# Yotsuei/ClearConverse

Hardware: AMD Instinct MI355X
Metric: xRT (audio-sec/wall-sec) end-to-end, 30 s 16 kHz clips (higher is better)
Workload: dtype bf16

## Files before the change

### clearconverse_amd/_lib.py

```python
from __future__ import annotations

import ctypes as C
import os
from pathlib import Path
from typing import Optional

_PKG = Path(__file__).resolve().parent
LIB_PATH = _PKG / "libccx.so"


class CcxError(RuntimeError):
    pass


class WhisperDims(C.Structure):
    _fields_ = [(n, C.c_int) for n in (
        "n_mels", "n_audio_ctx", "n_audio_state", "n_audio_head", "n_audio_layer",
        "n_vocab", "n_text_ctx", "n_text_state", "n_text_head", "n_text_layer")]


class SepformerDims(C.Structure):
    _fields_ = [(n, C.c_int) for n in (
        "n_filters", "kernel", "stride", "d_model", "n_head", "d_ffn", "n_layers", "n_blocks", "segment", "n_spk")]

# ... 41 lines not shown


class DecSeqState(C.Structure):
    _fields_ = [(n, C.c_int) for n in ("pos", "prompt_len", "n_gen", "done", "last_tok", "pen_tok", "last_ts_tok", "n_tokens")] + [
        ("sum_logprob", C.c_float), ("no_speech_prob", C.c_float)]


class DecSelectDesc(C.Structure):
    _fields_ = [
        ("logits", C.c_void_p), ("ld", C.c_int64), ("n_vocab", C.c_int), ("B", C.c_int),
        ("rules", C.POINTER(DecodeRules)), ("state", C.POINTER(DecSeqState)),
        ("prompt", C.POINTER(C.c_int)), ("max_prompt", C.c_int), ("sample_len", C.c_int),
        ("gen", C.POINTER(C.c_int)), ("cur_tok", C.POINTER(C.c_int)), ("pos", C.POINTER(C.c_int)), ("n_done", C.POINTER(C.c_int)),
        ("tok_emb", C.c_void_p), ("pos_emb", C.c_void_p), ("x", C.c_void_p), ("D", C.c_int),
        ("sample", C.c_int), ("temperature", C.c_float), ("seed", C.c_uint64), ("row0", C.c_int),
        ("logits_elems", C.c_int64), ("tok_emb_elems", C.c_int64), ("pos_emb_elems", C.c_int64), ("x_elems", C.c_int64),
        ("stream_ids", C.POINTER(C.c_int))]


class DecBeamDesc(C.Structure):
    _fields_ = [
        ("logits", C.c_void_p), ("ld", C.c_int64), ("n_vocab", C.c_int),
        ("G", C.c_int), ("beam_size", C.c_int), ("max_candidates", C.c_int),
        ("rules", C.POINTER(DecodeRules)), ("state", C.POINTER(DecSeqState)), ("sample_len", C.c_int),
        ("hist", C.POINTER(C.c_int)), ("cur_tok", C.POINTER(C.c_int)), ("pos", C.POINTER(C.c_int)), ("n_done", C.POINTER(C.c_int)),
        ("tok_emb", C.c_void_p), ("pos_emb", C.c_void_p), ("x", C.c_void_p), ("D", C.c_int),
        ("ind", C.POINTER(C.c_uint16)), ("ind_ld", C.c_int),
        ("fin_tok", C.POINTER(C.c_int)), ("fin_score", C.POINTER(C.c_float)), ("fin_n", C.POINTER(C.c_int)),
        ("fin_count", C.POINTER(C.c_int)),
        ("cand_id", C.POINTER(C.c_int)), ("cand_lp", C.POINTER(C.c_float)), ("tok_out", C.POINTER(C.c_int)),
        ("parent_out", C.POINTER(C.c_int)),
        ("logits_elems", C.c_int64), ("tok_emb_elems", C.c_int64), ("pos_emb_elems", C.c_int64), ("x_elems", C.c_int64)]


class BeamTrace(C.Structure):
    _fields_ = [("n_steps", C.c_int), ("cand_id", C.POINTER(C.c_int32)), ("cand_lp", C.POINTER(C.c_float)),
                ("tok", C.POINTER(C.c_int32)), ("parent", C.POINTER(C.c_int32)), ("score", C.POINTER(C.c_float))]


class DecTokenProbsDesc(C.Structure):
    _fields_ = [
        ("logits", C.c_void_p), ("logits_elems", C.c_int64), ("ld", C.c_int64), ("n_vocab", C.c_int), ("rows", C.c_int),
        ("lo", C.c_int), ("hi", C.c_int), ("pick", C.c_int),
        ("argmax", C.POINTER(C.c_int)), ("pick_prob", C.POINTER(C.c_float)),
        ("probs", C.c_void_p), ("probs_elems", C.c_int64)]


class DecPickProbsDesc(C.Structure):
    _fields_ = [
        ("logits", C.c_void_p), ("logits_elems", C.c_int64), ("ld", C.c_int64), ("rows", C.c_int), ("hi", C.c_int),
        ("picks", C.c_void_p), ("picks_elems", C.c_int64), ("pick_stride", C.c_int64),
        ("out", C.c_void_p), ("out_elems", C.c_int64), ("out_stride", C.c_int64)]


class SepDesc(C.Structure):
    _fields_ = (
        [(n, C.c_void_p) for n in ("h", "xin", "y", "qkv", "att", "feats", "fc")]
        + [(n, C.c_int64) for n in ("h_elems", "xin_elems", "y_elems", "qkv_elems", "att_elems", "feats_elems", "fc_elems")]
        + [("rows", C.c_int), ("seq_start", C.POINTER(C.c_int)), ("seq_len", C.POINTER(C.c_int)), ("n_seq", C.c_int),
           ("n_tok", C.c_int), ("d_ffn", C.c_int)]
        + [(n, C.c_void_p) for n in ("ln_g", "ln_b", "gln_g", "gln_b", "wqkv", "bqkv", "wo", "bo", "w1", "b1", "w2", "b2", "wdec")]
        + [(n, C.c_int64) for n in ("ln_elems", "gln_elems", "wqkv_elems", "bqkv_elems", "wo_elems", "bo_elems", "w1_elems",
                                    "b1_elems", "w2_elems", "b2_elems", "wdec_elems")]
        + [("utt_tok0", C.POINTER(C.c_int)), ("utt_L", C.POINTER(C.c_int)), ("utt_T", C.POINTER(C.c_int)), ("n_utt", C.c_int),
           ("segment", C.c_int), ("out", C.c_void_p), ("out_stride", C.c_int64), ("out_elems", C.c_int64)])


SEP_ATTN_BLOCK, SEP_ATTENTION, SEP_FFN, SEP_FINAL_NORM, SEP_DECODER = range(5)


class AlignDesc(C.Structure):
    _fields_ = [
        ("q", C.c_void_p), ("k", C.c_void_p), ("q_elems", C.c_int64), ("k_elems", C.c_int64),
        ("n_seq", C.c_int), ("H", C.c_int), ("Spad", C.c_int),
        ("heads", C.POINTER(C.c_int)), ("n_heads", C.c_int), ("head0", C.c_int), ("t", C.c_int),
        ("Hsel", C.c_int), ("T", C.c_int), ("Mmax", C.c_int),
        ("n_keys", C.POINTER(C.c_int)), ("n_rows", C.POINTER(C.c_int)), ("r0", C.c_int),
        ("P", C.c_void_p), ("A", C.c_void_p), ("P_elems", C.c_int64), ("A_elems", C.c_int64),
        ("text_idx", C.c_void_p), ("time_idx", C.c_void_p), ("path_len", C.c_void_p), ("jump_frame", C.c_void_p),
        ("text_idx_elems", C.c_int64), ("time_idx_elems", C.c_int64), ("path_len_elems", C.c_int64), ("jump_frame_elems", C.c_int64)]


ALIGN_SCORES, ALIGN_MATRIX, ALIGN_DTW = range(3)


_vp, _i, _i64, _f = C.c_void_p, C.c_int, C.c_int64, C.c_float
_ip = C.POINTER(C.c_int)
_i32p = C.POINTER(C.c_int32)
_i64p = C.POINTER(C.c_int64)
_fp = C.POINTER(C.c_float)

PROTOTYPES = {
    "ccx_version": (C.c_char_p, []),
    "ccx_ctx_create": (_i, [_i, C.POINTER(_vp)]),
    "ccx_ctx_destroy": (None, [_vp]),
    "ccx_last_error": (C.c_char_p, [_vp]),
    "ccx_prof_enable": (_i, [_vp, _i]),
    "ccx_prof_count": (_i, [_vp]),
    "ccx_prof_get": (_i, [_vp, _i, C.c_char_p, _i, C.POINTER(C.c_double), C.POINTER(C.c_double), _fp]),
    "ccx_gemm_bf16": (_i, [_vp, _i, _vp, _i64, _vp, _i64, _vp, _vp, _i64, _vp, _i64, _i, _i, _i, _vp]),
    "ccx_gemm_bf16_desc": (_i, [_vp, _i, C.POINTER(GemmDesc), _vp]),
    "ccx_layernorm": (_i, [_vp, _vp, _vp, _vp, _vp, _vp, _i, _i, _f, _vp]),
    "ccx_gather_rows": (_i, [_vp, _vp, _vp, _i, _i, _vp, _i64, _vp]),
    "ccx_peak_normalize": (_i, [_vp, _vp, _vp, _i64, _vp, _i, _f, _vp]),
    "ccx_row_variance": (_i, [_vp, _vp, _i64, _vp, _i, _vp, _vp]),
    "ccx_cross_attention_xa": (_i, [_vp, _vp, _vp, _vp, _vp, _vp, _vp, _i, _i, _i, _i, _i, _vp, _vp]),
    "ccx_cosine_rows": (_i, [_vp, _vp, _vp, _i, _i, _i, _vp, _vp]),
    "ccx_speaker_profiles": (_i, [_vp, _vp, _vp, _vp, _i, _i, _i, _i, _vp, _vp]),
    "ccx_resample_sinc": (_i, [_vp, _vp, _i64, _vp, _i, _i, _i, _i, _vp, _vp, _i64, _vp, _i, _vp]),
    "ccx_enc_attention": (_i, [_vp, _vp, _vp, _vp, _vp, _i, _i, _i, _i, _vp]),
    "ccx_whisper_create": (_i, [_vp, C.POINTER(WhisperDims), _i, C.POINTER(_vp)]),
    "ccx_whisper_destroy": (None, [_vp]),
    "ccx_whisper_set_tensor": (_i, [_vp, C.c_char_p, _vp, _i, _i, _i64p]),
    "ccx_whisper_set_max_audio": (_i, [_vp, C.c_double]),
    "ccx_whisper_share_encoder_scratch": (_i, [_vp, _vp]),
    "ccx_whisper_finalize": (_i, [_vp]),
    "ccx_whisper_set_rules": (_i, [_vp, C.POINTER(DecodeRules)]),
    "ccx_whisper_logmel": (_i, [_vp, _vp, _i64, _ip, _ip, _i, _vp, _vp]),
    "ccx_whisper_set_mel": (_i, [_vp, _vp, _i, _vp]),
    "ccx_whisper_encode": (_i, [_vp, _i, _vp, _vp]),
    "ccx_whisper_decoder_logits": (_i, [_vp, _i32p, _i, _i, _vp, _vp]),
    "ccx_whisper_decode_greedy": (_i, [_vp, _i32p, _i32p, _i, _i, _i, _i32p, _i32p, _fp, _fp, _vp]),
    "ccx_dec_attention_desc": (_i, [_vp, _i, C.POINTER(DecAttnDesc), _vp]),
    "ccx_dec_select_step": (_i, [_vp, C.POINTER(DecSelectDesc), _vp]),
    "ccx_dec_beam_step": (_i, [_vp, C.POINTER(DecBeamDesc), _vp]),
    "ccx_whisper_decode_beam": (_i, [_vp, _i32p, _i32p, _i, _i, _i32p, _i, _i, _i, _i, _i32p, _i32p, _fp, _i32p, _fp,
                                     C.POINTER(BeamTrace), _vp]),
    "ccx_dec_token_probs": (_i, [_vp, C.POINTER(DecTokenProbsDesc), _vp]),
    "ccx_dec_pick_probs": (_i, [_vp, C.POINTER(DecPickProbsDesc), _vp]),
    "ccx_align_op": (_i, [_vp, _i, C.POINTER(AlignDesc), _vp]),
    "ccx_whisper_align": (_i, [_vp, _i32p, _i32p, _i, _i, _i32p, _i32p, _i, _i, _vp, _vp, _i32p, _vp]),
    "ccx_whisper_align_probs": (_i, [_vp, _i32p, _i32p, _i, _i, _i32p, _i32p, _i, _i, _vp, _vp, _i32p, _i, _fp, _vp]),
    "ccx_whisper_last_cross_path": (_i, [_vp]),
    "ccx_whisper_set_sot_tail": (_i, [_vp, _i]),
    "ccx_whisper_detect_language": (_i, [_vp, _i, _i, _i, _i32p, _fp, _vp]),
    "ccx_whisper_prepare_lanes": (_i, [_vp, _vp]),
    "ccx_whisper_trace_lanes": (_i, [_vp, C.c_char_p, _i]),
    "ccx_whisper_decode": (_i, [_vp, _i32p, _i32p, _i, _i, _i, _f, C.c_uint64, _i32p, _i32p, _fp, _fp, _vp]),
    "ccx_whisper_decode_rows": (_i, [_vp, _i32p, _i32p, _i, _i, _i32p, _i, _i32p, _i, _f, C.c_uint64, _i32p, _i32p, _fp, _fp, _vp]),
    "ccx_sepformer_create": (_i, [_vp, C.POINTER(SepformerDims), _i, _i, C.POINTER(_vp)]),
    "ccx_sepformer_destroy": (None, [_vp]),
    "ccx_sepformer_set_tensor": (_i, [_vp, C.c_char_p, _vp, _i64]),
    "ccx_sepformer_finalize": (_i, [_vp]),
    "ccx_sepformer_separate": (_i, [_vp, _vp, _i64, _ip, _i, _vp, _vp]),
    "ccx_sep_op": (_i, [_vp, _i, C.POINTER(SepDesc), _vp]),
    "ccx_speaker_create": (_i, [_vp, _i, _i, _i, _i, _i64, C.POINTER(_vp)]),
    "ccx_speaker_destroy": (None, [_vp]),
    "ccx_speaker_set_tensor": (_i, [_vp, C.c_char_p, _vp, _i64]),
    "ccx_speaker_finalize": (_i, [_vp]),
    "ccx_speaker_embed": (_i, [_vp, _vp, _i64p, _ip, _i, _vp, _i64p, _ip, _vp, _vp]),
    "ccx_speaker_segment": (_i, [_vp, _vp, _i64p, _ip, _i, _vp, _i64, _ip, _vp]),
    "ccx_resnet_create": (_i, [_vp, _i, _i64, _i, C.POINTER(_vp)]),
    "ccx_resnet_destroy": (None, [_vp]),
    "ccx_resnet_set_tensor": (_i, [_vp, C.c_char_p, _vp, _i64]),
    "ccx_resnet_finalize": (_i, [_vp]),
    "ccx_resnet_embed": (_i, [_vp, _vp, _i64, _i, _i, _vp, _i, _ip, _i, _vp, _vp]),
    "ccx_specgate_create": (_i, [_vp, _i64, _i, _i, C.POINTER(_vp)]),
    "ccx_specgate_destroy": (None, [_vp]),
    "ccx_specgate_reduce": (_i, [_vp, _vp, _i64, _ip, _i, _f, _vp, _vp]),
    "ccx_specgate_reduce_long": (_i, [_vp, _vp, _i64, _f, _vp, _vp]),
    "ccx_specgate_set_clip_noise": (_i, [_vp, _i]),
}

_lib: Optional[C.CDLL] = None


def load() -> C.CDLL:
    global _lib
    if _lib is not None:
        return _lib
    if not LIB_PATH.exists():
        raise CcxError(f"{LIB_PATH} is missing: run `python -m clearconverse_amd.build` "
                       "(there is no CPU fallback for the HIP path)")
    import torch
    try:
        lib = C.CDLL(str(LIB_PATH))
    except OSError as e:
        raise CcxError(f"cannot load {LIB_PATH}: {e}") from e
    for name, (res, args) in PROTOTYPES.items():
        try:
            fn = getattr(lib, name)
        except AttributeError as e:
            raise CcxError(f"libccx.so does not export {name}") from e
        fn.restype = res
        fn.argtypes = args
    _lib = lib
    return lib


class Context:

    def __init__(self, device: int = 0):
        self.lib = load()
        h = _vp()
        rc = self.lib.ccx_ctx_create(device, C.byref(h))
        if rc != 0:
            raise CcxError(f"ccx_ctx_create({device}) failed: {self.lib.ccx_last_error(None).decode()}")
        self.handle = h
        self.device = device

    def check(self, rc: int, what: str = ""):
        if rc != 0:
            raise CcxError(f"{what or 'ccx call'} failed ({rc}): {self.lib.ccx_last_error(self.handle).decode()}")

    prof_on = False

    def prof_enable(self, on: bool = True):
        self.check(self.lib.ccx_prof_enable(self.handle, 1 if on else 0), "ccx_prof_enable")
        self.prof_on = bool(on)

    def prof_records(self):
        out = []
        buf = C.create_string_buffer(64)
        fl, by, ms = C.c_double(), C.c_double(), C.c_float()
        for i in range(self.lib.ccx_prof_count(self.handle)):
            self.check(self.lib.ccx_prof_get(self.handle, i, buf, 64, C.byref(fl), C.byref(by), C.byref(ms)), "ccx_prof_get")
            out.append((buf.value.decode(), fl.value, by.value, ms.value))
        return out

    def close(self):
        if getattr(self, "handle", None):
            self.lib.ccx_ctx_destroy(self.handle)
            self.handle = None

    def __del__(self):
        try:
            self.close()
        except Exception:
            pass


def current_stream_ptr() -> int:
    import torch
    return int(torch.cuda.current_stream().cuda_stream)


def ptr(t) -> int:
    if t is None:
        return 0
# ... 4 lines not shown
```

### clearconverse_amd/csrc/resnet.hip

```cpp
#include <string>
#include <vector>
#include <math.h>
#include "../../include/ccx.h"
#include "ccx_common.h"
#include "gemm_bf16.h"
#include "model_store.h"

namespace {

constexpr int FB_LEN = 400, FB_SHIFT = 160, FB_NFFT = 512, FB_MELS = 80, FB_MELW = 64;
constexpr int RN_C0 = 32, RN_EMB = 256, RN_STAGES = 4;
constexpr int RN_BLOCKS[RN_STAGES] = {3, 4, 6, 3};

__global__ __launch_bounds__(256) void fbank_kernel(const float* __restrict__ wav, long stride, int T, const float* __restrict__ window,
                                                    const float2* __restrict__ twiddle, const float* __restrict__ melw,
                                                    const int* __restrict__ mel_start, const int* __restrict__ mel_len,
                                                    float* __restrict__ feats_t) {
  __shared__ float2 buf[4][FB_NFFT];
  __shared__ float2 tw[FB_NFFT / 2];
  const int lane = threadIdx.x & 63, wave = threadIdx.x >> 6;
  for (int i = threadIdx.x; i < FB_NFFT / 2; i += 256) tw[i] = twiddle[i];
  const int chunk = blockIdx.y;
  const int t = blockIdx.x * 4 + wave;
  const bool live = t < T;
// ... 133 lines not shown
      const int row = idx / ((TW + 2) * 4), rem = idx - row * (TW + 2) * 4;
      const int px = rem >> 2, q = rem & 3;
      stg[it] = make_uint4(0, 0, 0, 0);
      if (idx < NCH && x0 + px < Wp) stg[it] = *(const uint4*)(src + ((long)row * Wp + x0 + px) * 32 + q * 8);
    }
    if (HAS_RESID) {
#pragma unroll
      for (int pt = 0; pt < 4; pt++) {
        const int x = x0 + pt * 16 + l15;
        rres[pt] = make_uint4(0, 0, 0, 0);
        if (x < W) rres[pt] = *(const uint4*)(resid + (orow + x) * 32 + 8 * hq);
      }
    }
  };
  auto put = [&]() {
#pragma unroll
    for (int it = 0; it < NIT; it++) {
      const int idx = tid + 256 * it;
      const int row = idx / ((TW + 2) * 4), rem = idx - row * (TW + 2) * 4;
      const int px = rem >> 2, q = rem & 3;
      if (idx < NCH) *(uint4*)(tile + (row * (TW + 2) + px) * PITCH + q * 16) = stg[it];
    }
  };
  fetch(0);
  bf16x8 wf[9][2];
#pragma unroll
  for (int t = 0; t < 9; t++)
#pragma unroll
    for (int j = 0; j < 2; j++) {
      const int co = 8 * (l15 >> 2) + 4 * j + (l15 & 3);
      wf[t][j] = *(const bf16x8*)(wpk + (long)co * 384 + (t / 3) * 128 + (t % 3) * 32 + hq * 8);
    }
  float bv[8];
#pragma unroll
  for (int i = 0; i < 8; i++) bv[i] = bias[8 * hq + i];
  const int n_tiles = (W + TW - 1) / TW;
  for (int k = 0; k < n_tiles; k++) {
    const int x0 = k * TW;
    put();
    uint4 rcur[4];
    if (HAS_RESID) {
#pragma unroll
      for (int pt = 0; pt < 4; pt++) rcur[pt] = rres[pt];
    }
    __syncthreads();
    if (k + 1 < n_tiles) fetch(x0 + TW);
    f32x4 acc[4][2];
#pragma unroll
    for (int pt = 0; pt < 4; pt++)
#pragma unroll
      for (int j = 0; j < 2; j++) acc[pt][j] = (f32x4){0.f, 0.f, 0.f, 0.f};
#pragma unroll
    for (int t = 0; t < 9; t++) {
      const int kh = t / 3, kw = t % 3;
#pragma unroll
      for (int pt = 0; pt < 4; pt++) {
        const bf16x8 bfrag = *(const bf16x8*)(tile + ((wave + kh) * (TW + 2) + pt * 16 + l15 + kw) * PITCH + hq * 16);
#pragma unroll
        for (int j = 0; j < 2; j++) acc[pt][j] = __builtin_amdgcn_mfma_f32_16x16x32_bf16(wf[t][j], bfrag, acc[pt][j], 0, 0, 0);
      }
    }
#pragma unroll
    for (int pt = 0; pt < 4; pt++) {
      const int x = x0 + pt * 16 + l15;
      if (x >= W) continue;
      float v[8];
#pragma unroll
      for (int j = 0; j < 2; j++)
#pragma unroll
        for (int r = 0; r < 4; r++) v[4 * j + r] = acc[pt][j][r] + bv[4 * j + r];
      const long off = (orow + x) * 32 + 8 * hq;
      if (HAS_RESID) {
        const uint32_t rw[4] = {rcur[pt].x, rcur[pt].y, rcur[pt].z, rcur[pt].w};
#pragma unroll
        for (int i = 0; i < 4; i++) {
          v[2 * i] += __uint_as_float(rw[i] << 16);
          v[2 * i + 1] += __uint_as_float(rw[i] & 0xffff0000u);
        }
      }
      uint4 o;
      o.x = pack_bf16x2(fmaxf(v[0], 0.f), fmaxf(v[1], 0.f)); o.y = pack_bf16x2(fmaxf(v[2], 0.f), fmaxf(v[3], 0.f));
      o.z = pack_bf16x2(fmaxf(v[4], 0.f), fmaxf(v[5], 0.f)); o.w = pack_bf16x2(fmaxf(v[6], 0.f), fmaxf(v[7], 0.f));
      *(uint4*)(out + off) = o;
    }
    __syncthreads();
  }
}

__global__ __launch_bounds__(256) void tstp_kernel(const bf16_t* __restrict__ act, int W4, const int* __restrict__ mask_chunk,
                                                   const float* __restrict__ weights, int n_w, float* __restrict__ pooled) {
  const int h = blockIdx.x, j = blockIdx.y, c = threadIdx.x;
  const int chunk = mask_chunk ? mask_chunk[j] : j;
  const long Wp = W4 + 2;
  const bf16_t* base = act + (((long)chunk * 12 + h + 1) * Wp + 1) * 256 + c;
  const float* wj = weights ? weights + (long)j * n_w : nullptr;
  float v1 = 0.f, v2 = 0.f, sx = 0.f;
  const float scale = (float)n_w / (float)W4;
  for (int t = 0; t < W4; t++) {
    const float w = wj ? wj[min((int)floorf(t * scale), n_w - 1)] : 1.f;
    v1 += w; v2 += w * w;
    sx = fmaf(w, bf16_to_f32(base[(long)t * 256]), sx);
  }
  v1 += 1e-8f;
  const float mean = sx / v1;
  float sq = 0.f;
  for (int t = 0; t < W4; t++) {
    const float w = wj ? wj[min((int)floorf(t * scale), n_w - 1)] : 1.f;
    const float d = bf16_to_f32(base[(long)t * 256]) - mean;
    sq = fmaf(w, d * d, sq);
  }
  const float var = sq / (v1 - v2 / v1 + 1e-8f);
  float* o = pooled + (long)j * 5120;
  o[c * 10 + h] = mean;
  o[2560 + c * 10 + h] = sqrtf(var);
}

__global__ __launch_bounds__(256) void embed_linear_kernel(const float* __restrict__ pooled, const float* __restrict__ W,
                                                           const float* __restrict__ bias, float* __restrict__ out) {
  const int lane = threadIdx.x & 63, o = blockIdx.x * 4 + (threadIdx.x >> 6), j = blockIdx.y;
  const float4* p = (const float4*)(pooled + (long)j * 5120);
  const float4* w = (const float4*)(W + (long)o * 5120);
  float s = 0.f;
  for (int i = lane; i < 5120 / 4; i += 64) {
    const float4 a = p[i], b = w[i];
    s += a.x * b.x + a.y * b.y + a.z * b.z + a.w * b.w;
  }
  s = wave_reduce_sum(s);
  if (lane == 0) out[(long)j * RN_EMB + o] = s + bias[o];
}

struct Conv {
  bf16_t* W = nullptr;
  float* b = nullptr;
  int cin = 0, cout = 0, k = 3, stride = 1, Kpad = 0;
};
struct Block {
  Conv c1, c2, sc;
  bool has_sc = false;
};

}

struct ccx_resnet {
  ccx_ctx* ctx = nullptr;
  int max_chunks = 0, max_masks = 0, max_frames = 0;
  long max_samples = 0;
  bool finalized = false;
  ccx_dev_store store{"resnet"};
  float *window = nullptr, *melw = nullptr;
  float2* twiddle = nullptr;
  int *mel_start = nullptr, *mel_len = nullptr;
  float *c1w = nullptr, *c1b = nullptr, *segW = nullptr, *segb = nullptr;
  std::vector<Block> blocks;
  float *feats_t = nullptr, *fmean = nullptr, *pooled = nullptr;
  bf16_t* act[RN_STAGES][3] = {};
  size_t act_elems[RN_STAGES] = {};
  int* mask_chunk_dev = nullptr;
  std::vector<int> mask_host[4];
  int mask_slot = 0;
  int last_T = -1;
  int halo_chunks = 0;
};

namespace {

int bn_fold(ccx_resnet* r, const std::string& name, int c, std::vector<float>& scale, std::vector<float>& shift) {
  CCX_NEED(r->store, g, name + ".weight", c); CCX_NEED(r->store, be, name + ".bias", c);
  CCX_NEED(r->store, rm, name + ".running_mean", c); CCX_NEED(r->store, rv, name + ".running_var", c);
  scale.resize(c); shift.resize(c);
  for (int i = 0; i < c; i++) {
    scale[i] = g->data[i] / sqrtf(rv->data[i] + 1e-5f);
    shift[i] = be->data[i] - rm->data[i] * scale[i];
  }
  return CCX_OK;
}

int load_conv(ccx_resnet* r, const std::string& wname, const std::string& bnname, int cin, int cout, int k, int stride, Conv& cv) {
  CCX_NEED(r->store, w, wname, (int64_t)cout * cin * k * k);
  std::vector<float> sc, sh;
  CCX_TRY(bn_fold(r, bnname, cout, sc, sh));
  cv.cin = cin; cv.cout = cout; cv.k = k; cv.stride = stride;
  cv.Kpad = ccx_align(k * cin, 64);
  std::vector<bf16_t> packed((size_t)cout * k * cv.Kpad, 0);
  for (int o = 0; o < cout; o++)
    for (int c = 0; c < cin; c++)
      for (int kh = 0; kh < k; kh++)
        for (int kw = 0; kw < k; kw++)
          packed[((size_t)o * k + kh) * cv.Kpad + kw * cin + c] = ccx_host_f32_to_bf16(w->data[(((size_t)o * cin + c) * k + kh) * k + kw] * sc[o]);
  CCX_TRY(r->store.upload(&cv.W, packed));
  CCX_TRY(r->store.upload(&cv.b, sh));
  return CCX_OK;
}

__global__ __launch_bounds__(256) void halo_zero_kernel(bf16_t* b0, bf16_t* b1, bf16_t* b2, int c0, int H, long Wp, int C) {
  bf16_t* buf = blockIdx.z == 0 ? b0 : (blockIdx.z == 1 ? b1 : b2);
  const int y = blockIdx.x;
  bf16_t* row = buf + (((long)(c0 + blockIdx.y) * (H + 2) + y) * Wp) * C;
  const uint4 z = make_uint4(0, 0, 0, 0);
  if (y == 0 || y == H + 1) {
    const long n = Wp * C / 8;
    for (long i = threadIdx.x; i < n; i += 256) ((uint4*)row)[i] = z;
  } else {
    const int n = C / 8;
    for (int i = threadIdx.x; i < 2 * n; i += 256) {
      bf16_t* cell = i < n ? row : row + (Wp - 1) * C;
      ((uint4*)cell)[i < n ? i : i - n] = z;
    }
  }
}

struct StageDims { int H, W, C; long Wp; };
void stage_dims(int T, StageDims (&d)[RN_STAGES]) {
  int H = FB_MELS, W = T, C = RN_C0;
  for (int s = 0; s < RN_STAGES; s++) {
    d[s] = {H, W, C, (long)W + 2};
    H /= 2; W = (W - 1) / 2 + 1; C *= 2;
  }
}

int run_conv(ccx_resnet* r, const Conv& cv, int epi, const bf16_t* in, const StageDims& di, bf16_t* out, const StageDims& dn,
             const bf16_t* resid, int n_chunks, hipStream_t st) {
  if (cv.cin == 32 && cv.cout == 32 && cv.k == 3 && cv.stride == 1 && di.H % 4 == 0 && (epi == EPI_BF16_RELU || epi == EPI_BF16_ADD_RELU)) {
    const dim3 grid(1, di.H / 4, n_chunks);
    {
      ccx_prof_scope ps(r->ctx, st, "conv3x3_c32_kernel", 2.0 * 9 * 32 * 32 * (double)n_chunks * di.H * di.W,
                        (double)n_chunks * di.H * di.W * 64.0 * (resid ? 3 : 2));
      if (resid) hipLaunchKernelGGL(conv3x3_c32_kernel<true>, grid, dim3(256), 0, st, in, cv.W, cv.b, resid, out, di.H, di.W);
      else hipLaunchKernelGGL(conv3x3_c32_kernel<false>, grid, dim3(256), 0, st, in, cv.W, cv.b, resid, out, di.H, di.W);
    }
    CCX_CHECK_LAUNCH(r->ctx);
    return CCX_OK;
  }
  GemmParams p;
  memset(&p, 0, sizeof(p));
  const int s = cv.stride;
  const int RI = (di.H + 2) / s;
  p.A = in + (cv.k == 1 ? (di.Wp + 1) * di.C : 0);
  p.lda = (long)s * di.C;
  p.K = cv.Kpad; p.ntaps = cv.k; p.a_tap_stride = di.Wp * di.C;
  p.W = cv.W; p.ldw = (long)cv.k * cv.Kpad;
  p.M = (int)((long)n_chunks * RI * di.Wp); p.N = cv.cout;
  p.bias = cv.b; p.out = out; p.ldo = cv.cout;
  p.rpb_in = (int)di.Wp; p.rpb_valid = dn.W; p.rpb_out = (int)dn.Wp; p.roff = (int)dn.Wp + 1;
  p.img_rows_in = RI; p.img_rows_valid = dn.H; p.img_rows_out = dn.H + 2;
  p.resid_bf16 = resid; p.ldrb = cv.cout;
  return ccx_launch_gemm(r->ctx, epi, p, st);
}

}

extern "C" {

int ccx_resnet_create(ccx_ctx* ctx, int max_chunks, int64_t max_samples, int max_masks, ccx_resnet** out) {
  if (!ctx || !out) return CCX_ERR_ARG;
  CCX_REQUIRE(ctx, max_chunks >= 1 && max_masks >= 1 && max_samples >= FB_LEN + 7 * FB_SHIFT, "resnet_create: bad capacities");
  const int max_frames = 1 + (int)((max_samples - FB_LEN) / FB_SHIFT);
  CCX_REQUIRE(ctx, (long)max_chunks * 82 * (max_frames + 2) < (1L << 31), "resnet_create: max_chunks x frames too large for one launch");
  ccx_resnet* r = new ccx_resnet();
  r->ctx = ctx; r->store.ctx = ctx; r->max_chunks = max_chunks; r->max_masks = max_masks; r->max_samples = max_samples;
  r->max_frames = max_frames;
  *out = r;
  return CCX_OK;
}

void ccx_resnet_destroy(ccx_resnet* r) {
  if (!r) return;
  r->store.free_all();
  delete r;
}

int ccx_resnet_set_tensor(ccx_resnet* r, const char* name, const float* data, int64_t numel) {
  if (!r) return CCX_ERR_ARG;
  CCX_REQUIRE(r->ctx, !r->finalized && name && data && numel > 0, "resnet: set_tensor bad arguments");
  return r->store.stage(name, data, numel);
}

int ccx_resnet_finalize(ccx_resnet* r) {
  if (!r) return CCX_ERR_ARG;
  ccx_ctx* ctx = r->ctx;
  CCX_REQUIRE(ctx, !r->finalized, "resnet: finalize called twice");
  {
    std::vector<float> win(FB_LEN);
    for (int i = 0; i < FB_LEN; i++) win[i] = (float)(0.54 - 0.46 * cos(2.0 * M_PI * i / (FB_LEN - 1)));
    std::vector<float2> tw(FB_NFFT / 2);
    for (int i = 0; i < FB_NFFT / 2; i++) tw[i] = make_float2((float)cos(-2.0 * M_PI * i / FB_NFFT), (float)sin(-2.0 * M_PI * i / FB_NFFT));
    auto mel = [](double f) { return 1127.0 * log(1.0 + f / 700.0); };
    const double mlo = mel(20.0), mhi = mel(8000.0), delta = (mhi - mlo) / (FB_MELS + 1);
    std::vector<float> mw((size_t)FB_MELS * FB_MELW, 0.f);
    std::vector<int> ms(FB_MELS, 0), ml(FB_MELS, 0);
    for (int m = 0; m < FB_MELS; m++) {
      const double left = mlo + m * delta, center = left + delta, right = center + delta;
      int first = -1, last = -1;
      std::vector<float> wts(FB_NFFT / 2, 0.f);
      for (int k = 0; k < FB_NFFT / 2; k++) {
        const double mk = mel(16000.0 / FB_NFFT * k);
        const double up = (mk - left) / (center - left), down = (right - mk) / (right - center);
        const double wv = fmax(0.0, fmin(up, down));
        wts[k] = (float)wv;
        if (wv > 0.0) { if (first < 0) first = k; last = k; }
      }
      if (first < 0) { first = 0; last = -1; }
      CCX_REQUIRE(ctx, last - first + 1 <= FB_MELW, "resnet: mel filter %d spans %d bins", m, last - first + 1);
      ms[m] = first; ml[m] = last - first + 1;
      for (int k = first; k <= last; k++) mw[(size_t)m * FB_MELW + (k - first)] = wts[k];
    }
    CCX_TRY(r->store.upload(&r->window, win)); CCX_TRY(r->store.upload(&r->twiddle, tw)); CCX_TRY(r->store.upload(&r->melw, mw));
    CCX_TRY(r->store.upload(&r->mel_start, ms)); CCX_TRY(r->store.upload(&r->mel_len, ml));
  }
  {
    CCX_NEED(r->store, w, "resnet.conv1.weight", RN_C0 * 9);
    std::vector<float> sc, sh;
    CCX_TRY(bn_fold(r, "resnet.bn1", RN_C0, sc, sh));
    std::vector<float> wf(RN_C0 * 9);
    for (int c = 0; c < RN_C0; c++)
      for (int k = 0; k < 9; k++) wf[c * 9 + k] = w->data[c * 9 + k] * sc[c];
    CCX_TRY(r->store.upload(&r->c1w, wf)); CCX_TRY(r->store.upload(&r->c1b, sh));
  }
  int cin = RN_C0;
  for (int s = 0; s < RN_STAGES; s++) {
    const int cout = RN_C0 << s;
    for (int b = 0; b < RN_BLOCKS[s]; b++) {
      const std::string p = "resnet.layer" + std::to_string(s + 1) + "." + std::to_string(b) + ".";
      const int stride = (s > 0 && b == 0) ? 2 : 1;
      Block blk;
      CCX_TRY(load_conv(r, p + "conv1.weight", p + "bn1", cin, cout, 3, stride, blk.c1));
      CCX_TRY(load_conv(r, p + "conv2.weight", p + "bn2", cout, cout, 3, 1, blk.c2));
      blk.has_sc = stride != 1 || cin != cout;
      if (blk.has_sc) CCX_TRY(load_conv(r, p + "shortcut.0.weight", p + "shortcut.1", cin, cout, 1, stride, blk.sc));
      r->blocks.push_back(blk);
      cin = cout;
    }
  }
  {
    CCX_NEED(r->store, w, "resnet.seg_1.weight", (int64_t)RN_EMB * 5120); CCX_NEED(r->store, b, "resnet.seg_1.bias", RN_EMB);
    CCX_TRY(r->store.upload(&r->segW, w->data)); CCX_TRY(r->store.upload(&r->segb, b->data));
  }
  r->store.staged.clear();
  const int T = r->max_frames;
  CCX_TRY(r->store.alloc(&r->feats_t, (size_t)r->max_chunks * FB_MELS * T, true));
  CCX_TRY(r->store.alloc(&r->fmean, (size_t)r->max_chunks * FB_MELS, true));
  CCX_TRY(r->store.alloc(&r->pooled, (size_t)r->max_masks * 5120, true));
  CCX_TRY(r->store.alloc(&r->mask_chunk_dev, (size_t)r->max_masks, true));
  StageDims d[RN_STAGES];
  stage_dims(T, d);
  for (int s = 0; s < RN_STAGES; s++) {
    r->act_elems[s] = (size_t)r->max_chunks * (d[s].H + 2) * d[s].Wp * d[s].C + 4 * d[s].Wp * d[s].C + 1024;
    for (int k = 0; k < 3; k++) CCX_TRY(r->store.alloc(&r->act[s][k], r->act_elems[s], true));
  }
  r->finalized = true;
  return CCX_OK;
}

int ccx_resnet_embed(ccx_resnet* r, const float* wav_dev, int64_t stride, int n_samples, int n_chunks, const float* weights_dev,
                     int n_w, const int* mask_chunk, int n_masks, float* out_dev, void* stream_) {
  if (!r) return CCX_ERR_ARG;
  ccx_ctx* ctx = r->ctx;
  hipStream_t st = (hipStream_t)stream_;
  CCX_REQUIRE(ctx, r->finalized, "resnet: not finalized");
  CCX_REQUIRE(ctx, wav_dev && out_dev && n_chunks >= 1 && n_chunks <= r->max_chunks, "resnet_embed: bad chunk count %d (max %d)", n_chunks, r->max_chunks);
  CCX_REQUIRE(ctx, n_samples <= stride && n_samples <= r->max_samples, "resnet_embed: n_samples %d exceeds stride or capacity", n_samples);
  const int T = n_samples >= FB_LEN ? 1 + (n_samples - FB_LEN) / FB_SHIFT : 0;
  StageDims d[RN_STAGES];
  stage_dims(T > 0 ? T : 1, d);
  CCX_REQUIRE(ctx, T >= 1 && d[3].W >= 2, "resnet_embed: %d samples are too short (at least two pooled frames are needed)", n_samples);
  if (weights_dev) {
    CCX_REQUIRE(ctx, mask_chunk && n_masks >= 1 && n_masks <= r->max_masks && n_w >= 1, "resnet_embed: bad mask arguments");
    for (int j = 0; j < n_masks; j++)
      CCX_REQUIRE(ctx, mask_chunk[j] >= 0 && mask_chunk[j] < n_chunks, "resnet_embed: mask_chunk[%d]=%d out of range", j, mask_chunk[j]);
    std::vector<int>& keep = r->mask_host[r->mask_slot++ & 3];
    keep.assign(mask_chunk, mask_chunk + n_masks);
    CCX_HIP(ctx, hipMemcpyAsync(r->mask_chunk_dev, keep.data(), (size_t)n_masks * 4, hipMemcpyHostToDevice, st));
  } else {
    n_masks = n_chunks;
    CCX_REQUIRE(ctx, n_masks <= r->max_masks, "resnet_embed: %d chunks exceed the mask capacity %d", n_masks, r->max_masks);
  }
  if (T != r->last_T) { r->last_T = T; r->halo_chunks = 0; }
  if (n_chunks > r->halo_chunks) {
    for (int s = 0; s < RN_STAGES; s++)
      hipLaunchKernelGGL(halo_zero_kernel, dim3(d[s].H + 2, n_chunks - r->halo_chunks, 3), dim3(256), 0, st, r->act[s][0], r->act[s][1],
                         r->act[s][2], r->halo_chunks, d[s].H, d[s].Wp, d[s].C);
    CCX_CHECK_LAUNCH(ctx);
    r->halo_chunks = n_chunks;
  }
  {
    ccx_prof_scope ps(ctx, st, "fbank_kernel", 0.0, (double)n_chunks * n_samples * 4 + (double)n_chunks * T * FB_MELS * 4);
    hipLaunchKernelGGL(fbank_kernel, dim3(ccx_cdiv(T, 4), n_chunks), dim3(256), 0, st, wav_dev, (long)stride, T, r->window, r->twiddle,
                       r->melw, r->mel_start, r->mel_len, r->feats_t);
  }
  CCX_CHECK_LAUNCH(ctx);
  hipLaunchKernelGGL(fbank_mean_kernel, dim3(n_chunks * FB_MELS), dim3(256), 0, st, r->feats_t, T, r->fmean);
  CCX_CHECK_LAUNCH(ctx);
  {
    ccx_prof_scope ps(ctx, st, "conv1_kernel", 2.0 * 9 * RN_C0 * (double)n_chunks * FB_MELS * T,
                      (double)n_chunks * FB_MELS * T * (4 + RN_C0 * 2));
    hipLaunchKernelGGL(conv1_kernel, dim3(ccx_cdiv(T, 256), FB_MELS, n_chunks), dim3(256), 0, st, r->feats_t, r->fmean, T, r->c1w, r->c1b,
                       r->act[0][0]);
  }
  CCX_CHECK_LAUNCH(ctx);
  int bi = 0, cur = 0;
  const bf16_t* x = r->act[0][0];
  int xs = 0;
  for (int s = 0; s < RN_STAGES; s++) {
    for (int b = 0; b < RN_BLOCKS[s]; b++, bi++) {
      const Block& blk = r->blocks[bi];
      bf16_t* tbuf; bf16_t* ybuf; bf16_t* scbuf = nullptr;
      if (xs == s) {
        tbuf = r->act[s][(cur + 1) % 3]; ybuf = r->act[s][(cur + 2) % 3];
      } else {
        tbuf = r->act[s][0]; ybuf = r->act[s][1]; scbuf = r->act[s][2];
      }
      CCX_TRY(run_conv(r, blk.c1, EPI_BF16_RELU, x, d[xs], tbuf, d[s], nullptr, n_chunks, st));
      const bf16_t* resid = x;
      if (blk.has_sc) {
        CCX_REQUIRE(ctx, scbuf != nullptr, "resnet: shortcut convolution inside a stage");
        CCX_TRY(run_conv(r, blk.sc, EPI_BF16, x, d[xs], scbuf, d[s], nullptr, n_chunks, st));
        resid = scbuf;
      }
      CCX_TRY(run_conv(r, blk.c2, EPI_BF16_ADD_RELU, tbuf, d[s], ybuf, d[s], resid, n_chunks, st));
      x = ybuf; xs = s;
      cur = (int)(ybuf == r->act[s][0] ? 0 : (ybuf == r->act[s][1] ? 1 : 2));
    }
  }
  hipLaunchKernelGGL(tstp_kernel, dim3(10, n_masks), dim3(256), 0, st, x, d[3].W, weights_dev ? r->mask_chunk_dev : nullptr, weights_dev,
                     n_w, r->pooled);
  CCX_CHECK_LAUNCH(ctx);
  hipLaunchKernelGGL(embed_linear_kernel, dim3(RN_EMB / 4, n_masks), dim3(256), 0, st, r->pooled, r->segW, r->segb, out_dev);
  CCX_CHECK_LAUNCH(ctx);
  return CCX_OK;
}

}
```

### include/ccx.h

```cpp
#ifndef CCX_H
#define CCX_H
#include <stdint.h>
#ifdef __cplusplus
extern "C" {
#endif

#define CCX_DTYPE_F32 0
#define CCX_DTYPE_BF16 1
#define CCX_DTYPE_F16 2

typedef struct ccx_ctx ccx_ctx;
typedef struct ccx_whisper ccx_whisper;

const char* ccx_version(void);
int ccx_ctx_create(int device, ccx_ctx** out);
void ccx_ctx_destroy(ccx_ctx* ctx);
const char* ccx_last_error(const ccx_ctx* ctx);

int ccx_prof_enable(ccx_ctx* ctx, int on);
int ccx_prof_count(ccx_ctx* ctx);
int ccx_prof_get(ccx_ctx* ctx, int i, char* name_out, int name_cap, double* flops, double* bytes, float* ms);


int ccx_gemm_bf16(ccx_ctx* ctx, int epi, const void* A_dev, int64_t lda, const void* W_dev, int64_t ldw,
// ... 198 lines not shown
  const int* n_keys;
  const int* n_rows;
  int r0;
  void* P; void* A;
  int64_t P_elems, A_elems;
  void* text_idx; void* time_idx; void* path_len; void* jump_frame;
  int64_t text_idx_elems, time_idx_elems, path_len_elems, jump_frame_elems;
} ccx_align_desc;

int ccx_align_op(ccx_ctx* ctx, int op, const ccx_align_desc* desc, void* stream);

int ccx_whisper_align(ccx_whisper* w, const int32_t* tokens, const int32_t* lens, int max_len, int B, const int32_t* n_frames,
                      const int32_t* heads, int n_heads, int row0, float* probs_out_dev, float* matrix_out_dev,
                      int32_t* jump_frame_out, void* stream);
int ccx_whisper_align_probs(ccx_whisper* w, const int32_t* tokens, const int32_t* lens, int max_len, int B, const int32_t* n_frames,
                            const int32_t* heads, int n_heads, int row0, float* probs_out_dev, float* matrix_out_dev,
                            int32_t* jump_frame_out, int prob_hi, float* token_prob_out, void* stream);

int ccx_whisper_last_cross_path(ccx_whisper* w);

int ccx_whisper_set_sot_tail(ccx_whisper* w, int n_tail);
int ccx_whisper_detect_language(ccx_whisper* w, int B, int lang_begin, int n_lang, int32_t* lang_token_out, float* probs_out,
                                void* stream);

int ccx_whisper_prepare_lanes(ccx_whisper* w, void* stream);
int ccx_whisper_trace_lanes(ccx_whisper* w, const char* path, int level);


typedef struct ccx_sepformer ccx_sepformer;
typedef struct {
  int n_filters, kernel, stride, d_model, n_head, d_ffn, n_layers, n_blocks, segment, n_spk;
} ccx_sepformer_dims;

int ccx_sepformer_create(ccx_ctx* ctx, const ccx_sepformer_dims* dims, int max_tokens, int max_utts,
                         ccx_sepformer** out);
void ccx_sepformer_destroy(ccx_sepformer* s);
int ccx_sepformer_set_tensor(ccx_sepformer* s, const char* name, const float* data, int64_t numel);
int ccx_sepformer_finalize(ccx_sepformer* s);
int ccx_sepformer_separate(ccx_sepformer* s, const float* mix_dev, int64_t stride, const int* n_samples, int B,
                           float* out_dev, void* stream);

#define CCX_SEP_ATTN_BLOCK 0
#define CCX_SEP_ATTENTION 1
#define CCX_SEP_FFN 2
#define CCX_SEP_FINAL_NORM 3
#define CCX_SEP_DECODER 4

typedef struct ccx_sep_desc {
  void* h; const void* xin; void* y; const void* qkv; void* att; const void* feats; const void* fc;
  int64_t h_elems, xin_elems, y_elems, qkv_elems, att_elems, feats_elems, fc_elems;
  int rows;
  const int* seq_start; const int* seq_len; int n_seq;
  int n_tok, d_ffn;
  const void* ln_g; const void* ln_b; const void* gln_g; const void* gln_b;
  const void* wqkv; const void* bqkv; const void* wo; const void* bo;
  const void* w1; const void* b1; const void* w2; const void* b2; const void* wdec;
  int64_t ln_elems, gln_elems, wqkv_elems, bqkv_elems, wo_elems, bo_elems, w1_elems, b1_elems, w2_elems, b2_elems, wdec_elems;
  const int* utt_tok0; const int* utt_L; const int* utt_T; int n_utt; int segment;
  void* out; int64_t out_stride; int64_t out_elems;
} ccx_sep_desc;

int ccx_sep_op(ccx_ctx* ctx, int op, const ccx_sep_desc* desc, void* stream);


typedef struct ccx_speaker ccx_speaker;
int ccx_speaker_create(ccx_ctx* ctx, int kind, int n_classes, int powerset, int max_crops, int64_t max_samples,
                       ccx_speaker** out);
void ccx_speaker_destroy(ccx_speaker* s);
int ccx_speaker_set_tensor(ccx_speaker* s, const char* name, const float* data, int64_t numel);
int ccx_speaker_finalize(ccx_speaker* s);
int ccx_speaker_embed(ccx_speaker* s, const float* wav_dev, const int64_t* offsets, const int* n_samples, int n,
                      const float* weights_dev, const int64_t* w_offsets, const int* w_lens, float* out_dev, void* stream);
int ccx_speaker_segment(ccx_speaker* s, const float* wav_dev, const int64_t* offsets, const int* n_samples, int n,
                        float* out_dev, int64_t out_capacity_rows, int* frames_out, void* stream);

typedef struct ccx_resnet ccx_resnet;
int ccx_resnet_create(ccx_ctx* ctx, int max_chunks, int64_t max_samples, int max_masks, ccx_resnet** out);
void ccx_resnet_destroy(ccx_resnet* r);
int ccx_resnet_set_tensor(ccx_resnet* r, const char* name, const float* data, int64_t numel);
int ccx_resnet_finalize(ccx_resnet* r);
int ccx_resnet_embed(ccx_resnet* r, const float* wav_dev, int64_t stride, int n_samples, int n_chunks, const float* weights_dev,
                     int n_w, const int* mask_chunk, int n_masks, float* out_dev, void* stream);

typedef struct ccx_specgate ccx_specgate;
int ccx_specgate_create(ccx_ctx* ctx, int64_t max_samples, int max_clips, int sample_rate, ccx_specgate** out);
void ccx_specgate_destroy(ccx_specgate* g);
int ccx_specgate_reduce(ccx_specgate* g, const float* y_dev, int64_t stride, const int* n_samples, int B,
                        float prop_decrease, float* out_dev, void* stream);
int ccx_specgate_set_clip_noise(ccx_specgate* g, int on);
int ccx_specgate_reduce_long(ccx_specgate* g, const float* y_dev, int64_t n, float prop_decrease, float* out_dev, void* stream);

#ifdef __cplusplus
}
#endif
#endif
```

Baseline: 1749.

## Add direct MFMA 3x3 conv kernel for 64-channel ResNet layers

Adds a persistent direct 3x3 convolution kernel for 64->64 channel ResNet stage convs. It keeps the weights in registers (AGPRs), stages a padded input tile in LDS with software prefetch of the next tile, and fuses bias, residual add and ReLU into the epilogue, replacing the implicit-GEMM path for these layers. It is enabled by default and can be turned off with an env var. It also adds a standalone test entry point. The risks are register pressure and LDS occupancy limits, and the grid is capped at the CU count.

```diff
diff --git a/clearconverse_amd/_lib.py b/clearconverse_amd/_lib.py
--- a/clearconverse_amd/_lib.py
+++ b/clearconverse_amd/_lib.py
@@ -147,6 +147,17 @@
 
 
 ALIGN_SCORES, ALIGN_MATRIX, ALIGN_DTW = range(3)
+
+
+class Conv3x3Desc(C.Structure):
+    _fields_ = [
+        ("inp", C.c_void_p), ("w", C.c_void_p), ("bias", C.c_void_p), ("resid", C.c_void_p), ("out", C.c_void_p),
+        ("n_chunks", C.c_int), ("H", C.c_int), ("W", C.c_int), ("cin", C.c_int), ("cout", C.c_int),
+        ("in_elems", C.c_int64), ("w_elems", C.c_int64), ("bias_elems", C.c_int64), ("resid_elems", C.c_int64),
+        ("out_elems", C.c_int64)]
+
+
+CONV_GEMM, CONV_DIRECT = range(2)
 
 
 _vp, _i, _i64, _f = C.c_void_p, C.c_int, C.c_int64, C.c_float
@@ -220,6 +231,7 @@
     "ccx_resnet_set_tensor": (_i, [_vp, C.c_char_p, _vp, _i64]),
     "ccx_resnet_finalize": (_i, [_vp]),
     "ccx_resnet_embed": (_i, [_vp, _vp, _i64, _i, _i, _vp, _i, _ip, _i, _vp, _vp]),
+    "ccx_resnet_conv3x3": (_i, [_vp, _i, C.POINTER(Conv3x3Desc), _vp]),
     "ccx_specgate_create": (_i, [_vp, _i64, _i, _i, C.POINTER(_vp)]),
     "ccx_specgate_destroy": (None, [_vp]),
     "ccx_specgate_reduce": (_i, [_vp, _vp, _i64, _ip, _i, _f, _vp, _vp]),
diff --git a/clearconverse_amd/csrc/resnet.hip b/clearconverse_amd/csrc/resnet.hip
--- a/clearconverse_amd/csrc/resnet.hip
+++ b/clearconverse_amd/csrc/resnet.hip
@@ -239,6 +239,162 @@
       o.x = pack_bf16x2(fmaxf(v[0], 0.f), fmaxf(v[1], 0.f)); o.y = pack_bf16x2(fmaxf(v[2], 0.f), fmaxf(v[3], 0.f));
       o.z = pack_bf16x2(fmaxf(v[4], 0.f), fmaxf(v[5], 0.f)); o.w = pack_bf16x2(fmaxf(v[6], 0.f), fmaxf(v[7], 0.f));
       *(uint4*)(out + off) = o;
+    }
+    __syncthreads();
+  }
+}
+
+constexpr int C64_TH = 4, C64_TW = 64, C64_PITCH = 160;
+template <bool HAS_RESID, bool RAGGED>
+__global__ __launch_bounds__(256) void conv3x3_c64_kernel(const bf16_t* __restrict__ in, const bf16_t* __restrict__ wpk,
+                                                          const float* __restrict__ bias, const bf16_t* __restrict__ resid,
+                                                          bf16_t* __restrict__ out, int H, int W, int n_strips) {
+  constexpr int TH = C64_TH, TW = C64_TW, PITCH = C64_PITCH, NPT = TW / 16;
+  __shared__ __attribute__((aligned(16))) char tile[(TH + 2) * (TW + 2) * PITCH];
+  const int tid = threadIdx.x, lane = tid & 63;
+  const int wave = __builtin_amdgcn_readfirstlane(tid >> 6);
+  const int cg = wave & 1, rg = wave >> 1;
+  const int l15 = lane & 15, hq = lane >> 4;
+  const long Wp = W + 2;
+  const int strips = H / TH;
+  const int G = gridDim.x, gb = xcd_remap(blockIdx.x, G);
+  const int n_tiles = (W + TW - 1) / TW;
+  const int total = gb < n_strips ? (n_strips - gb + G - 1) / G * n_tiles : 0;
+  struct Loc { long row0; int x0; };
+  auto locate = [&](int t) {
+    const int i = t / n_tiles, k = t - i * n_tiles, g = gb + i * G;
+    const int img = g / strips, y0 = (g - img * strips) * TH;
+    return Loc{(long)img * (H + 2) + y0, RAGGED ? k * TW : min(k * TW, W - TW)};
+  };
+  constexpr int NCH = (TH + 2) * (TW + 2) * 8, NIT = (NCH + 255) / 256;
+  uint4 stg[NIT];
+  uint4 rres[2][NPT];
+  const int cbase = 32 * cg + 8 * hq;
+  auto fetch = [&](int t) {
+    const Loc L = locate(t);
+    const bf16_t* src = in + L.row0 * Wp * 64;
+#pragma unroll
+    for (int it = 0; it < NIT; it++) {
+      const int idx = tid + 256 * it;
+      const int row = idx / ((TW + 2) * 8), rem = idx - row * (TW + 2) * 8;
+      const int px = rem >> 3, q = rem & 7;
+      stg[it] = make_uint4(0, 0, 0, 0);
+      if (idx < NCH && (!RAGGED || L.x0 + px < Wp)) stg[it] = *(const uint4*)(src + ((long)row * Wp + L.x0 + px) * 64 + q * 8);
+    }
+    if (HAS_RESID) {
+#pragma unroll
+      for (int rr = 0; rr < 2; rr++)
+#pragma unroll
+        for (int pt = 0; pt < NPT; pt++) {
+          const int x = L.x0 + pt * 16 + l15;
+          rres[rr][pt] = make_uint4(0, 0, 0, 0);
+          if (!RAGGED || x < W) rres[rr][pt] = *(const uint4*)(resid + ((L.row0 + 2 * rg + rr + 1) * Wp + 1 + x) * 64 + cbase);
+        }
+    }
+  };
+  auto put = [&]() {
+#pragma unroll
+    for (int it = 0; it < NIT; it++) {
+      const int idx = tid + 256 * it;
+      const int row = idx / ((TW + 2) * 8), rem = idx - row * (TW + 2) * 8;
+      const int px = rem >> 3, q = rem & 7;
+      if (idx < NCH) *(uint4*)(tile + (row * (TW + 2) + px) * PITCH + q * 16) = stg[it];
+    }
+  };
+  if (!RAGGED && total > 0) fetch(0);
+  bf16x8 wf[3][6][2];
+#pragma unroll
+  for (int kh = 0; kh < 3; kh++)
+#pragma unroll
+    for (int c = 0; c < 6; c++)
+#pragma unroll
+      for (int j = 0; j < 2; j++) {
+        const int co = 32 * cg + 8 * (l15 >> 2) + 4 * j + (l15 & 3);
+        wf[kh][c][j] = *(const bf16x8*)(wpk + (long)co * 576 + kh * 192 + c * 32 + hq * 8);
+      }
+#pragma unroll
+  for (int kh = 0; kh < 3; kh++)
+#pragma unroll
+    for (int c = 0; c < 6; c++)
+#pragma unroll
+      for (int j = 0; j < 2; j++) asm volatile("" : "+a"(wf[kh][c][j]));
+  float bv[8];
+#pragma unroll
+  for (int i = 0; i < 8; i++) bv[i] = bias[cbase + i];
+#pragma unroll
+  for (int i = 0; i < 8; i++) asm volatile("" ::"v"(bv[i]));
+  constexpr int SPLIT = NPT > 2 ? 3 : 1, NC = 6 / SPLIT, NSTEP = 6 * SPLIT;
+  auto frags = [&](int s, bf16x8 (&f)[NC][NPT]) {
+    const int rk = s / SPLIT, c0 = (s % SPLIT) * NC;
+    const int trow = 2 * rg + rk / 3 + rk % 3;
+#pragma unroll
+    for (int c = 0; c < NC; c++)
+#pragma unroll
+      for (int pt = 0; pt < NPT; pt++)
+        f[c][pt] = *(const bf16x8*)(tile + (trow * (TW + 2) + pt * 16 + l15 + ((c0 + c) >> 1)) * PITCH + ((c0 + c) & 1) * 64 + hq * 16);
+  };
+  for (int t = 0; t < total; t++) {
+    const Loc L = locate(t);
+    const int x0 = L.x0;
+    const long orow = (L.row0 + 2 * rg + 1) * Wp + 1;
+    if (RAGGED) fetch(t);
+    put();
+    uint4 rcur[2][NPT];
+    if (HAS_RESID) {
+#pragma unroll
+      for (int rr = 0; rr < 2; rr++)
+#pragma unroll
+        for (int pt = 0; pt < NPT; pt++) rcur[rr][pt] = rres[rr][pt];
+    }
+    __syncthreads();
+    if (!RAGGED && t + 1 < total) fetch(t + 1);
+    bf16x8 fr[2][NC][NPT];
+    f32x4 acc[2][NPT][2];
+    frags(0, fr[0]);
+#pragma unroll
+    for (int s = 0; s < NSTEP; s++) {
+      const int rk = s / SPLIT, c0 = (s % SPLIT) * NC;
+      const int rr = rk / 3, kh = rk % 3;
+      if (s + 1 < NSTEP) frags(s + 1, fr[(s + 1) & 1]);
+      __builtin_amdgcn_sched_barrier(0);
+      if (kh == 0 && c0 == 0) {
+#pragma unroll
+        for (int pt = 0; pt < NPT; pt++)
+#pragma unroll
+          for (int j = 0; j < 2; j++) acc[rr][pt][j] = (f32x4){0.f, 0.f, 0.f, 0.f};
+      }
+#pragma unroll
+      for (int c = 0; c < NC; c++)
+#pragma unroll
+        for (int pt = 0; pt < NPT; pt++)
+#pragma unroll
+          for (int j = 0; j < 2; j++)
+            acc[rr][pt][j] = __builtin_amdgcn_mfma_f32_16x16x32_bf16(wf[kh][c0 + c][j], fr[s & 1][c][pt], acc[rr][pt][j], 0, 0, 0);
+      if (kh == 2 && c0 + NC == 6) {
+#pragma unroll
+        for (int pt = 0; pt < NPT; pt++) {
+          const int x = x0 + pt * 16 + l15;
+          if (RAGGED && x >= W) continue;
+          float v[8];
+#pragma unroll
+          for (int j = 0; j < 2; j++)
+#pragma unroll
+            for (int r = 0; r < 4; r++) v[4 * j + r] = acc[rr][pt][j][r] + bv[4 * j + r];
+          if (HAS_RESID) {
+            const uint32_t rw[4] = {rcur[rr][pt].x, rcur[rr][pt].y, rcur[rr][pt].z, rcur[rr][pt].w};
+#pragma unroll
+            for (int i = 0; i < 4; i++) {
+              v[2 * i] += __uint_as_float(rw[i] << 16);
+              v[2 * i + 1] += __uint_as_float(rw[i] & 0xffff0000u);
+            }
+          }
+          uint4 o;
+          o.x = pack_bf16x2(fmaxf(v[0], 0.f), fmaxf(v[1], 0.f)); o.y = pack_bf16x2(fmaxf(v[2], 0.f), fmaxf(v[3], 0.f));
+          o.z = pack_bf16x2(fmaxf(v[4], 0.f), fmaxf(v[5], 0.f)); o.w = pack_bf16x2(fmaxf(v[6], 0.f), fmaxf(v[7], 0.f));
+          *(uint4*)(out + (orow + rr * Wp + x) * 64 + cbase) = o;
+        }
+      }
+      __builtin_amdgcn_sched_barrier(0);
     }
     __syncthreads();
   }
@@ -317,6 +473,7 @@
   int mask_slot = 0;
   int last_T = -1;
   int halo_chunks = 0;
+  int direct = 0;
 };
 
 namespace {
@@ -375,17 +532,36 @@
   }
 }
 
-int run_conv(ccx_resnet* r, const Conv& cv, int epi, const bf16_t* in, const StageDims& di, bf16_t* out, const StageDims& dn,
+enum { DIRECT_C32 = 1, DIRECT_C64 = 2 };
+
+int run_conv(ccx_ctx* ctx, int direct, const Conv& cv, int epi, const bf16_t* in, const StageDims& di, bf16_t* out, const StageDims& dn,
              const bf16_t* resid, int n_chunks, hipStream_t st) {
-  if (cv.cin == 32 && cv.cout == 32 && cv.k == 3 && cv.stride == 1 && di.H % 4 == 0 && (epi == EPI_BF16_RELU || epi == EPI_BF16_ADD_RELU)) {
+  const bool relu3x3 = cv.k == 3 && cv.stride == 1 && (epi == EPI_BF16_RELU || epi == EPI_BF16_ADD_RELU);
+  if ((direct & DIRECT_C32) && relu3x3 && cv.cin == 32 && cv.cout == 32 && di.H % 4 == 0) {
     const dim3 grid(1, di.H / 4, n_chunks);
     {
-      ccx_prof_scope ps(r->ctx, st, "conv3x3_c32_kernel", 2.0 * 9 * 32 * 32 * (double)n_chunks * di.H * di.W,
+      ccx_prof_scope ps(ctx, st, "conv3x3_c32_kernel", 2.0 * 9 * 32 * 32 * (double)n_chunks * di.H * di.W,
                         (double)n_chunks * di.H * di.W * 64.0 * (resid ? 3 : 2));
       if (resid) hipLaunchKernelGGL(conv3x3_c32_kernel<true>, grid, dim3(256), 0, st, in, cv.W, cv.b, resid, out, di.H, di.W);
       else hipLaunchKernelGGL(conv3x3_c32_kernel<false>, grid, dim3(256), 0, st, in, cv.W, cv.b, resid, out, di.H, di.W);
     }
-    CCX_CHECK_LAUNCH(r->ctx);
+    CCX_CHECK_LAUNCH(ctx);
+    return CCX_OK;
+  }
+  if ((direct & DIRECT_C64) && relu3x3 && cv.cin == 64 && cv.cout == 64 && di.H % C64_TH == 0 && resid != out) {
+    const int n_strips = n_chunks * (di.H / C64_TH);
+    int n_cu = 0;
+    CCX_HIP(ctx, hipDeviceGetAttribute(&n_cu, hipDeviceAttributeMultiprocessorCount, ctx->device));
+    const dim3 grid(n_strips < n_cu ? n_strips : n_cu);
+    const bool ragged = di.W < C64_TW;
+    {
+      ccx_prof_scope ps(ctx, st, "conv3x3_c64_kernel", 2.0 * 9 * 64 * 64 * (double)n_chunks * di.H * di.W,
+                        (double)n_chunks * di.H * di.W * 128.0 * (resid ? 3 : 2));
+      auto k = resid ? (ragged ? conv3x3_c64_kernel<true, true> : conv3x3_c64_kernel<true, false>)
+                     : (ragged ? conv3x3_c64_kernel<false, true> : conv3x3_c64_kernel<false, false>);
+      hipLaunchKernelGGL(k, grid, dim3(256), 0, st, in, cv.W, cv.b, resid, out, di.H, di.W, n_strips);
+    }
+    CCX_CHECK_LAUNCH(ctx);
     return CCX_OK;
   }
   GemmParams p;
@@ -401,7 +577,7 @@
   p.rpb_in = (int)di.Wp; p.rpb_valid = dn.W; p.rpb_out = (int)dn.Wp; p.roff = (int)dn.Wp + 1;
   p.img_rows_in = RI; p.img_rows_valid = dn.H; p.img_rows_out = dn.H + 2;
   p.resid_bf16 = resid; p.ldrb = cv.cout;
-  return ccx_launch_gemm(r->ctx, epi, p, st);
+  return ccx_launch_gemm(ctx, epi, p, st);
 }
 
 }
@@ -416,6 +592,8 @@
   ccx_resnet* r = new ccx_resnet();
   r->ctx = ctx; r->store.ctx = ctx; r->max_chunks = max_chunks; r->max_masks = max_masks; r->max_samples = max_samples;
   r->max_frames = max_frames;
+  const char* e = getenv("CCX_RESNET_DIRECT_C64");
+  r->direct = DIRECT_C32 | ((e && atoi(e) == 0) ? 0 : DIRECT_C64);
   *out = r;
   return CCX_OK;
 }
@@ -566,14 +744,14 @@
       } else {
         tbuf = r->act[s][0]; ybuf = r->act[s][1]; scbuf = r->act[s][2];
       }
-      CCX_TRY(run_conv(r, blk.c1, EPI_BF16_RELU, x, d[xs], tbuf, d[s], nullptr, n_chunks, st));
+      CCX_TRY(run_conv(ctx, r->direct, blk.c1, EPI_BF16_RELU, x, d[xs], tbuf, d[s], nullptr, n_chunks, st));
       const bf16_t* resid = x;
       if (blk.has_sc) {
         CCX_REQUIRE(ctx, scbuf != nullptr, "resnet: shortcut convolution inside a stage");
-        CCX_TRY(run_conv(r, blk.sc, EPI_BF16, x, d[xs], scbuf, d[s], nullptr, n_chunks, st));
+        CCX_TRY(run_conv(ctx, r->direct, blk.sc, EPI_BF16, x, d[xs], scbuf, d[s], nullptr, n_chunks, st));
         resid = scbuf;
       }
-      CCX_TRY(run_conv(r, blk.c2, EPI_BF16_ADD_RELU, tbuf, d[s], ybuf, d[s], resid, n_chunks, st));
+      CCX_TRY(run_conv(ctx, r->direct, blk.c2, EPI_BF16_ADD_RELU, tbuf, d[s], ybuf, d[s], resid, n_chunks, st));
       x = ybuf; xs = s;
       cur = (int)(ybuf == r->act[s][0] ? 0 : (ybuf == r->act[s][1] ? 1 : 2));
     }
@@ -586,4 +764,38 @@
   return CCX_OK;
 }
 
-}
+int ccx_resnet_conv3x3(ccx_ctx* ctx, int form, const ccx_conv3x3_desc* d, void* stream) {
+  if (!ctx) return CCX_ERR_ARG;
+  CCX_REQUIRE(ctx, d != nullptr, "ccx_resnet_conv3x3: desc is NULL");
+  CCX_REQUIRE(ctx, form == CCX_CONV_GEMM || form == CCX_CONV_DIRECT, "ccx_resnet_conv3x3: unknown form %d", form);
+  CCX_REQUIRE(ctx, d->in && d->w && d->bias && d->out, "ccx_resnet_conv3x3: in / w / bias / out must not be NULL");
+  CCX_REQUIRE(ctx, d->out != d->in && d->out != d->resid, "ccx_resnet_conv3x3: out must not alias in or resid");
+  CCX_REQUIRE(ctx, d->n_chunks >= 1 && d->H >= 1 && d->W >= 1, "ccx_resnet_conv3x3: empty problem (%d chunks of %d x %d)", d->n_chunks, d->H, d->W);
+  CCX_REQUIRE(ctx, d->cin >= 32 && d->cin % 32 == 0 && d->cout >= 16 && d->cout % 16 == 0,
+              "ccx_resnet_conv3x3: cin=%d must be a multiple of 32 and cout=%d a multiple of 16", d->cin, d->cout);
+  const long Wp = (long)d->W + 2, rows = (long)d->n_chunks * (d->H + 2) * Wp;
+  CCX_REQUIRE(ctx, rows < (1L << 31), "ccx_resnet_conv3x3: %ld padded pixels are too many for one launch", rows);
+  for (const void* p : {d->in, d->w, d->out, d->resid}) CCX_REQUIRE(ctx, ((uintptr_t)p & 15) == 0, "ccx_resnet_conv3x3: buffers must be 16-byte aligned");
+  Conv cv;
+  cv.W = (bf16_t*)d->w; cv.b = (float*)d->bias; cv.cin = d->cin; cv.cout = d->cout; cv.k = 3; cv.stride = 1;
+  cv.Kpad = ccx_align(3 * d->cin, 64);
+  CCX_REQUIRE(ctx, (long)d->cout * 3 * cv.Kpad <= d->w_elems && d->cout <= d->bias_elems,
+              "ccx_resnet_conv3x3: w needs %ld elements (w_elems=%ld), bias %d (bias_elems=%ld)", (long)d->cout * 3 * cv.Kpad, (long)d->w_elems,
+              d->cout, (long)d->bias_elems);
+  long in_need = rows * d->cin;
+  if (form == CCX_CONV_GEMM) in_need = (rows - 1) * d->cin + 2 * Wp * d->cin + cv.Kpad;
+  CCX_REQUIRE(ctx, in_need <= d->in_elems, "ccx_resnet_conv3x3: in is read up to element %ld, in_elems=%ld", in_need, (long)d->in_elems);
+  CCX_REQUIRE(ctx, rows * d->cout <= d->out_elems, "ccx_resnet_conv3x3: out is written up to element %ld, out_elems=%ld", rows * d->cout,
+              (long)d->out_elems);
+  CCX_REQUIRE(ctx, !d->resid || rows * d->cout <= d->resid_elems, "ccx_resnet_conv3x3: resid is read up to element %ld, resid_elems=%ld",
+              rows * d->cout, (long)d->resid_elems);
+  if (form == CCX_CONV_DIRECT)
+    CCX_REQUIRE(ctx, d->cin == 64 && d->cout == 64 && d->H % C64_TH == 0,
+                "ccx_resnet_conv3x3: the direct form takes 64 -> 64 channels and H a multiple of %d (cin=%d cout=%d H=%d)", C64_TH, d->cin,
+                d->cout, d->H);
+  const StageDims dd = {d->H, d->W, d->cin, Wp};
+  return run_conv(ctx, form == CCX_CONV_DIRECT ? DIRECT_C64 : 0, cv, d->resid ? EPI_BF16_ADD_RELU : EPI_BF16_RELU, (const bf16_t*)d->in, dd,
+                  (bf16_t*)d->out, dd, (const bf16_t*)d->resid, d->n_chunks, (hipStream_t)stream);
+}
+
+}
diff --git a/include/ccx.h b/include/ccx.h
--- a/include/ccx.h
+++ b/include/ccx.h
@@ -304,6 +304,16 @@
 int ccx_resnet_embed(ccx_resnet* r, const float* wav_dev, int64_t stride, int n_samples, int n_chunks, const float* weights_dev,
                      int n_w, const int* mask_chunk, int n_masks, float* out_dev, void* stream);
 
+typedef struct ccx_conv3x3_desc {
+  const void* in; const void* w; const void* bias; const void* resid;
+  const void* out;
+  int n_chunks, H, W, cin, cout;
+  int64_t in_elems, w_elems, bias_elems, resid_elems, out_elems;
+} ccx_conv3x3_desc;
+enum { CCX_CONV_GEMM = 0,
+       CCX_CONV_DIRECT = 1    };
+int ccx_resnet_conv3x3(ccx_ctx* ctx, int form, const ccx_conv3x3_desc* desc, void* stream);
+
 typedef struct ccx_specgate ccx_specgate;
 int ccx_specgate_create(ccx_ctx* ctx, int64_t max_samples, int max_clips, int sample_rate, ccx_specgate** out);
 void ccx_specgate_destroy(ccx_specgate* g);
```

New measurement: 1760, median of 6. About the same (+0.7%).
